# mit-han-lab/distrifuser

Measured on AMD Instinct MI355X. Metric: end-to-end latency (s) per image, SDXL 50-step DDIM, lower is better.
Workload: dtype bf16; 1 GPU; model=sdxl-base (random init), global_batch=1, image=3840x3840, seq_len=230400, scheduler=ddim, steps_per_image=50, parallelism=patch1, mode=corrected_async_gn, cuda_graph=True

## Files before the change

### distrifuser_amd/csrc/attention.hip

```cpp

#include "common.h"
#include "kernels.h"

#include <algorithm>
#include <type_traits>

namespace {

constexpr int QW = 32;
constexpr int KVB = 128;
constexpr bool SPLIT_STAGE = true;

typedef float float4v_ __attribute__((ext_vector_type(4)));
typedef float float16v __attribute__((ext_vector_type(16)));
typedef short short4v __attribute__((ext_vector_type(4)));
typedef __attribute__((address_space(3))) short4v lds_short4v;

template <int DPAD>
__device__ __forceinline__ int v_swz(int t) {
    if constexpr (DPAD % 128 == 0)
        return (t & 3) << 6;
    else if constexpr (DPAD % 64 == 0)
        return ((t >> 1) & 1) << 6;
    else
        return 0;
}

__device__ __forceinline__ uint32_t cvt_pk_bf16(float a, float b) {
    uint32_t r;
    asm("v_cvt_pk_bf16_f32 %0, %1, %2" : "=v"(r) : "v"(a), "v"(b));
    return r;
}

__device__ __forceinline__ void lds_barrier() {
    asm volatile("s_waitcnt lgkmcnt(0)\n\ts_barrier" ::: "memory");
}

__device__ __forceinline__ float half_max(float v) {
    const uint32_t u = __builtin_bit_cast(uint32_t, v);
    const auto r = __builtin_amdgcn_permlane32_swap(u, u, false, false);
    const uint32_t a = r[0], b = r[1];
    float m;
    asm("v_max_f32 %0, %1, %2" : "=v"(m) : "v"(a), "v"(b));
    return m;
}
__device__ __forceinline__ float half_sum(float v) {
    const uint32_t u = __builtin_bit_cast(uint32_t, v);
    const auto r = __builtin_amdgcn_permlane32_swap(u, u, false, false);
    const uint32_t a = r[0], b = r[1];
    return __builtin_bit_cast(float, a) + __builtin_bit_cast(float, b);
}

template <int NW, int DPAD, bool DFULL, bool SPLIT, bool LSE>
__global__ __launch_bounds__(NW * WAVE_SIZE)
__attribute__((amdgpu_waves_per_eu(DPAD == 64 ? 4 : 2))) void flash_attn_kernel(
    std::conditional_t<LSE, FlashAttnLseParams, FlashAttnParams> p, bool off32) {
    constexpr int NT = NW * WAVE_SIZE;
    constexpr int QBLK = QW * NW;
    constexpr int K_ROW = DPAD * 2 + 8;
    constexpr int V_ROW = DPAD * 2;
    constexpr int KS = DPAD / 16;
    constexpr int DT = DPAD / 32;
    constexpr int KCOLS = DPAD / 8;
    constexpr int NLD = KVB * KCOLS / NT;
    static_assert(KVB * KCOLS % NT == 0);
    __shared__ __attribute__((aligned(16))) char k_lds[KVB * K_ROW];
    __shared__ __attribute__((aligned(16))) char v_lds[KVB * V_ROW];

    const int tid = threadIdx.x;
    const int wave = tid / WAVE_SIZE;
    const int lane = tid % WAVE_SIZE;
    const int lo = lane & 31;
    const int hi = lane >> 5;

    const int bh = blockIdx.y;
    const int b = bh / p.H;
    const int h = bh % p.H;
    const int64_t q0 = (int64_t)blockIdx.x * QBLK;

    const int LC = (int)p.LC;
    const int Lkv = (int)(p.NC * p.LC);
    const uint16_t* qbase = p.q + b * p.q_sb + h * p.q_sh;
    const uint16_t* kbase = p.k + b * p.k_sb + h * p.k_sh;
    const uint16_t* vbase = p.v + b * p.v_sb + h * p.v_sh;

    short8 qf[KS];
    const int64_t qrow = q0 + wave * QW + lo;
    const bool qvalid = qrow < p.Lq;
    {
        const uint16_t* qp = qbase + (qvalid ? qrow : (p.Lq - 1)) * p.q_sl;
#pragma unroll
        for (int ks = 0; ks < KS; ++ks) {
            const int d0 = ks * 16 + hi * 8;
            if (DFULL || d0 + 8 <= p.Dh)
                qf[ks] = *reinterpret_cast<const short8*>(qp + d0);
            else
                qf[ks] = short8{0, 0, 0, 0, 0, 0, 0, 0};
        }
    }

    int vrd[DT];
    {
        const int i = lane & 15;
        const int q = i >> 2;
        const int col_b = ((lane >> 4) & 1) * 32 + (i & 3) * 8;
#pragma unroll
        for (int dt = 0; dt < DT; ++dt)
            vrd[dt] = (hi * 8 + q) * V_ROW + ((dt * 64 + col_b) ^ v_swz<DPAD>(q));
    }

    int cur_chunk = 0, cur_tin = 0;
    const char* kcur = reinterpret_cast<const char*>(kbase);
    const char* vcur = reinterpret_cast<const char*>(vbase);
    int tile_lo = 0, tile_hi = 0;
    if constexpr (LSE) {
        const int n_tiles = (Lkv + KVB - 1) / KVB;
        const int n_splits = (int)gridDim.z, split = (int)blockIdx.z;
        tile_lo = (int)((int64_t)split * n_tiles / n_splits);
        tile_hi = (int)((int64_t)(split + 1) * n_tiles / n_splits);
        if (tile_lo > 0) {
            const int tok = tile_lo * KVB;
            cur_chunk = tok / LC;
            cur_tin = tok - cur_chunk * LC;
            kcur = reinterpret_cast<const char*>(kbase + cur_chunk * p.k_sc + cur_tin * p.k_sl);
            vcur = reinterpret_cast<const char*>(vbase + cur_chunk * p.v_sc + cur_tin * p.v_sl);
        }
    }
    uint4 kreg[NLD], vreg[NLD];
    constexpr bool ROWPASS = NT % KCOLS == 0;
    auto stage_row = [&](int i) {
        if constexpr (ROWPASS)
            return tid / KCOLS + i * (NT / KCOLS);
        else
            return (tid + i * NT) / KCOLS;
    };
    auto stage_col = [&](int i) {
        if constexpr (ROWPASS)
            return tid % KCOLS;
        else
            return (tid + i * NT) % KCOLS;
    };
    auto stage_d_ok = [&](int i) { return DFULL || stage_col(i) * 8 + 8 <= p.Dh; };
    const uint32_t koff = (uint32_t)stage_row(0) * ((uint32_t)p.k_sl * 2) + stage_col(0) * 16;
    const uint32_t voff = (uint32_t)stage_row(0) * ((uint32_t)p.v_sl * 2) + stage_col(0) * 16;
    const int k_pass = (NT / KCOLS) * (int)p.k_sl * 2;
    const int v_pass = (NT / KCOLS) * (int)p.v_sl * 2;
    auto tile_rsrc = [](const char* cur) {
        return __builtin_amdgcn_make_buffer_rsrc(const_cast<char*>(cur), 0, 0xFFFFFFFFu,
                                                 0x00020000);
    };
    auto stage_load = [&](int t0, bool full) {
        if (ROWPASS && full && off32 && cur_tin + KVB <= LC) {
            const auto krs = tile_rsrc(kcur);
            const auto vrs = tile_rsrc(vcur);
#pragma unroll
            for (int i = 0; i < NLD; ++i) {
                if constexpr (!DFULL) {
                    kreg[i] = uint4{0, 0, 0, 0};
                    vreg[i] = uint4{0, 0, 0, 0};
                }
                if (stage_d_ok(i)) {
                    kreg[i] = __builtin_bit_cast(
                        uint4, __builtin_amdgcn_raw_buffer_load_b128(
                                   krs, (int)koff, i * k_pass, 0));
                    vreg[i] = __builtin_bit_cast(
                        uint4, __builtin_amdgcn_raw_buffer_load_b128(
                                   vrs, (int)voff, i * v_pass, 0));
                }
            }
        } else {
#pragma unroll
            for (int i = 0; i < NLD; ++i) {
                const int t_local = stage_row(i);
                const int d8 = stage_col(i);
                int tin = cur_tin + t_local;
                int ch = cur_chunk;
                while (tin >= LC) {
                    tin -= LC;
                    ++ch;
                }
                kreg[i] = uint4{0, 0, 0, 0};
                vreg[i] = uint4{0, 0, 0, 0};
                if (stage_d_ok(i) && t0 + t_local < Lkv) {
                    kreg[i] = *reinterpret_cast<const uint4*>(
                        kbase + ch * p.k_sc + tin * p.k_sl + d8 * 8);
                    vreg[i] = *reinterpret_cast<const uint4*>(
                        vbase + ch * p.v_sc + tin * p.v_sl + d8 * 8);
                }
            }
        }
        cur_tin += KVB;
        kcur += KVB * p.k_sl * 2;
        vcur += KVB * p.v_sl * 2;
        if (cur_tin >= LC) {
            do {
                cur_tin -= LC;
                ++cur_chunk;
            } while (cur_tin >= LC);
            kcur = reinterpret_cast<const char*>(kbase + cur_chunk * p.k_sc + cur_tin * p.k_sl);
            vcur = reinterpret_cast<const char*>(vbase + cur_chunk * p.v_sc + cur_tin * p.v_sl);
        }
    };
    auto stage_write = [&]() {
#pragma unroll
        for (int i = 0; i < NLD; ++i) {
            const int t_local = stage_row(i);
            const int d8 = stage_col(i);
            char* kdst = &k_lds[t_local * K_ROW + d8 * 16];
            *reinterpret_cast<uint2*>(kdst) = uint2{kreg[i].x, kreg[i].y};
            *reinterpret_cast<uint2*>(kdst + 8) = uint2{kreg[i].z, kreg[i].w};
            *reinterpret_cast<uint4*>(
                &v_lds[t_local * V_ROW + ((d8 * 16) ^ v_swz<DPAD>(t_local))]) = vreg[i];
        }
    };

    float m_raw = -1e30f;
    float msc = -1e30f;
    float l_run = 0.f;
    float16v ot[DT] = {};
    const float scale2 = p.scale * 1.44269504088896340736f;
    const float defer_raw = 11.0f / scale2;

    auto qk_tile = [&](int st) {
        float16v s = {};
        __builtin_amdgcn_s_setprio(1);
#pragma unroll
        for (int ks = 0; ks < KS; ++ks) {
            const int t = st * 32 + lo;
            const char* ksrc = &k_lds[t * K_ROW + (ks * 16 + hi * 8) * 2];
            const uint2 k0 = *reinterpret_cast<const uint2*>(ksrc);
            const uint2 k1 = *reinterpret_cast<const uint2*>(ksrc + 8);
            const uint4 kk{k0.x, k0.y, k1.x, k1.y};
            const short8 kfrag = __builtin_bit_cast(short8, kk);
            s = __builtin_amdgcn_mfma_f32_32x32x16_bf16(kfrag, qf[ks], s, 0, 0, 0);
        }
        __builtin_amdgcn_s_setprio(0);
        return s;
    };

    auto compute = [&]<int NST, bool MASK>(int t0) {
        float16v s_cur = qk_tile(0);
#pragma unroll
        for (int st = 0; st < NST; ++st) {
            float16v s_nxt;
            if (st + 1 < NST) s_nxt = qk_tile(st + 1);
            const float16v s = s_cur;
            float tm = -1e30f;
            float pv[16];
#pragma unroll
            for (int r = 0; r < 16; ++r) {
                float v = s[r];
                if (MASK) {
                    const int crow = (r & 3) + 8 * (r >> 2) + 4 * hi;
                    if (t0 + st * 32 + crow >= Lkv) v = -1e30f;
                }
                pv[r] = v;
                tm = fmaxf(tm, v);
            }
            tm = half_max(tm);

            if (__any(m_raw == -1e30f || tm > m_raw + defer_raw)) {
                const float m_new = fmaxf(m_raw, tm);
                const float msc_new = m_new * scale2;
                const float corr = __builtin_amdgcn_exp2f(msc - msc_new);
                m_raw = m_new;
                msc = msc_new;
                l_run *= corr;
#pragma unroll
                for (int dt = 0; dt < DT; ++dt)
#pragma unroll
                    for (int r = 0; r < 16; ++r) ot[dt][r] *= corr;
            }
            float tsum = 0.f;
#pragma unroll
            for (int r = 0; r < 16; ++r) {
                pv[r] = __builtin_amdgcn_exp2f(__builtin_fmaf(pv[r], scale2, -msc));
                tsum += pv[r];
            }
            l_run += half_sum(tsum);

            uint32_t w[8];
#pragma unroll
            for (int i = 0; i < 8; ++i) w[i] = cvt_pk_bf16(pv[2 * i], pv[2 * i + 1]);
            short8 pb[2];
#pragma unroll
            for (int kt = 0; kt < 2; ++kt) {
                const auto r0 = __builtin_amdgcn_permlane32_swap(w[4 * kt + 0], w[4 * kt + 2],
                                                                 false, false);
                const auto r1 = __builtin_amdgcn_permlane32_swap(w[4 * kt + 1], w[4 * kt + 3],
                                                                 false, false);
                const uint4 pw{r0[0], r1[0], r0[1], r1[1]};
                pb[kt] = __builtin_bit_cast(short8, pw);
            }

            __builtin_amdgcn_s_setprio(1);
#pragma unroll
            for (int dt = 0; dt < DT; ++dt) {
#pragma unroll
                for (int kt = 0; kt < 2; ++kt) {
                    const char* vsrc = &v_lds[vrd[dt] + (st * 32 + kt * 16) * V_ROW];
                    const short4v v0 =
                        __builtin_amdgcn_ds_read_tr16_b64_v4i16((lds_short4v*)vsrc);
                    const short4v v1 =
                        __builtin_amdgcn_ds_read_tr16_b64_v4i16((lds_short4v*)(vsrc + 4 * V_ROW));
                    const short8 vf = __builtin_shufflevector(v0, v1, 0, 1, 2, 3, 4, 5, 6, 7);
                    ot[dt] = __builtin_amdgcn_mfma_f32_32x32x16_bf16(vf, pb[kt], ot[dt], 0, 0, 0);
                }
            }
            __builtin_amdgcn_s_setprio(0);
            s_cur = s_nxt;
        }
    };

    const int tile0 = LSE ? tile_lo : 0;
    const int n_full = LSE ? min(tile_hi, Lkv / KVB) : Lkv / KVB;
    const int rem = LSE && tile_hi * KVB <= Lkv ? 0 : Lkv % KVB;
    if (Lkv > 0) {
        stage_load(tile0 * KVB, tile0 < n_full);
        stage_write();
        lds_barrier();
    }
    __builtin_amdgcn_s_waitcnt(0x0F70);
    for (int tile = tile0; tile < n_full; ++tile) {
        const int t0 = tile * KVB;
        const bool next_full = tile + 1 < n_full;
        auto load_next = [&]() {
            if (next_full || rem) stage_load(t0 + KVB, next_full);
        };
        if (SPLIT) load_next();
        compute.template operator()<KVB / 32, false>(t0);
        if (next_full || rem) {
            lds_barrier();
            if (!SPLIT) load_next();
            stage_write();
            lds_barrier();
        }
    }
    if (rem == 64)
        compute.template operator()<2, false>(n_full * KVB);
    else if (rem)
        compute.template operator()<KVB / 32, true>(n_full * KVB);

    const float inv = l_run > 0.f ? 1.f / l_run : 0.f;
    if constexpr (LSE) {
        const float lse = l_run > 0.f
                              ? 0.69314718055994530942f * (msc + __builtin_amdgcn_logf(l_run))
                              : -__builtin_inff();
        const int64_t sb = (int64_t)blockIdx.z * p.B + b;
        if (qvalid && hi == 0) p.lse[(sb * p.H + h) * p.Lq + qrow] = lse;
        if (p.o_part != nullptr) {
            float* op32 = p.o_part + (sb * p.Lq + (qvalid ? qrow : 0)) * (p.H * p.Dh) +
                          (int64_t)h * p.Dh;
#pragma unroll
            for (int dt = 0; dt < DT; ++dt) {
#pragma unroll
                for (int g = 0; g < 4; ++g) {
                    const int d0 = dt * 32 + 8 * g + 4 * hi;
                    if (qvalid && (DFULL || d0 + 4 <= p.Dh))
                        *reinterpret_cast<float4*>(op32 + d0) =
                            float4{ot[dt][4 * g] * inv, ot[dt][4 * g + 1] * inv,
                                   ot[dt][4 * g + 2] * inv, ot[dt][4 * g + 3] * inv};
                }
            }
            return;
        }
    }
    uint16_t* op = p.o + ((int64_t)b * p.Lq + (qvalid ? qrow : 0)) * (p.H * p.Dh) +
                   (int64_t)h * p.Dh;
#pragma unroll
    for (int dt = 0; dt < DT; ++dt) {
        uint32_t ow[8];
#pragma unroll
        for (int i = 0; i < 8; ++i) {
            const uint32_t e0 =
                __builtin_bit_cast(uint16_t, __float2bfloat16(ot[dt][2 * i] * inv));
            const uint32_t e1 =
                __builtin_bit_cast(uint16_t, __float2bfloat16(ot[dt][2 * i + 1] * inv));
            ow[i] = e0 | (e1 << 16);
        }
#pragma unroll
        for (int g = 0; g < 4; g += 2) {
            const auto rx = __builtin_amdgcn_permlane32_swap(ow[2 * g], ow[2 * g + 2],
                                                             false, false);
            const auto ry = __builtin_amdgcn_permlane32_swap(ow[2 * g + 1], ow[2 * g + 3],
                                                             false, false);
            const int d0 = dt * 32 + 8 * (g + hi);
            if (qvalid && (DFULL || d0 + 8 <= p.Dh))
                *reinterpret_cast<uint4*>(op + d0) = uint4{rx[0], ry[0], rx[1], ry[1]};
        }
    }
}

}

namespace {

template <bool OUT_BF16>
__global__ __launch_bounds__(256) void merge_attn_kernel(MergeAttnParams p) {
    const int dcols = p.Dh / 8;
    const int64_t idx = (int64_t)blockIdx.x * 256 + threadIdx.x;
    const int64_t rows = (int64_t)p.B * p.Lq * p.H;
    if (idx >= rows * dcols) return;
    const int64_t row = idx / dcols;
    const int dc = (int)(idx - row * dcols);
    const int h = (int)(row % p.H);
    const int64_t bq = row / p.H;
    const int64_t qi = bq % p.Lq;
    const int64_t b = bq / p.Lq;
    const int64_t lse_row = (b * p.H + h) * p.Lq + qi;
    const int64_t lse_ss = (int64_t)p.B * p.H * p.Lq;
    const int64_t o_ss = rows * p.Dh;

    float m = -__builtin_inff();
    for (int s = 0; s < p.S; ++s) m = fmaxf(m, p.lse_parts[s * lse_ss + lse_row]);
    float acc[8] = {};
    float wsum = 0.f;
    if (m > -__builtin_inff()) {
        const float* src = p.o_parts + row * p.Dh + dc * 8;
        for (int s = 0; s < p.S; ++s) {
            const float w = expf(p.lse_parts[s * lse_ss + lse_row] - m);
            const float4 a = *reinterpret_cast<const float4*>(src + s * o_ss);
            const float4 c = *reinterpret_cast<const float4*>(src + s * o_ss + 4);
            if (w > 0.f) {
                wsum += w;
                acc[0] += w * a.x, acc[1] += w * a.y, acc[2] += w * a.z, acc[3] += w * a.w;
                acc[4] += w * c.x, acc[5] += w * c.y, acc[6] += w * c.z, acc[7] += w * c.w;
            }
        }
        const float inv = 1.f / wsum;
#pragma unroll
        for (int j = 0; j < 8; ++j) acc[j] *= inv;
    }
    if (OUT_BF16) {
        uint32_t w[4];
#pragma unroll
        for (int j = 0; j < 4; ++j) {
            const uint32_t e0 = __builtin_bit_cast(uint16_t, __float2bfloat16(acc[2 * j]));
            const uint32_t e1 = __builtin_bit_cast(uint16_t, __float2bfloat16(acc[2 * j + 1]));
            w[j] = e0 | (e1 << 16);
        }
        *reinterpret_cast<uint4*>(static_cast<uint16_t*>(p.out) + row * p.Dh + dc * 8) =
            uint4{w[0], w[1], w[2], w[3]};
    } else {
        float* dst = static_cast<float*>(p.out) + row * p.Dh + dc * 8;
        *reinterpret_cast<float4*>(dst) = float4{acc[0], acc[1], acc[2], acc[3]};
        *reinterpret_cast<float4*>(dst + 4) = float4{acc[4], acc[5], acc[6], acc[7]};
    }
    if (dc == 0 && p.lse != nullptr)
        p.lse[lse_row] = wsum > 0.f ? m + logf(wsum) : -__builtin_inff();
}

}

void launch_merge_attention(const MergeAttnParams& p, hipStream_t stream) {
    const int64_t total = (int64_t)p.B * p.Lq * p.H * (p.Dh / 8);
    if (total == 0) return;
    const dim3 grid((unsigned)((total + 255) / 256));
    if (p.out_bf16)
        merge_attn_kernel<true><<<grid, 256, 0, stream>>>(p);
    else
        merge_attn_kernel<false><<<grid, 256, 0, stream>>>(p);
}

namespace {

template <int DPAD>
bool fits_off32(const FlashAttnParams& p) {
    const int64_t sl = p.k_sl > p.v_sl ? p.k_sl : p.v_sl;
    return sl >= 0 && sl * 2 * KVB + DPAD * 2 <= (int64_t)INT32_MAX;
}

template <int DPAD>
void launch_dpad_lse(const FlashAttnLseParams& p, int splits, hipStream_t stream) {
    constexpr int NW = 8;
    const int qblk = QW * NW;
    dim3 grid((unsigned)((p.Lq + qblk - 1) / qblk), (unsigned)(p.B * p.H), (unsigned)splits);
    dim3 block(NW * WAVE_SIZE);
    const bool off32 = fits_off32<DPAD>(p);
    if (p.Dh == DPAD)
        flash_attn_kernel<NW, DPAD, true, SPLIT_STAGE, true><<<grid, block, 0, stream>>>(p, off32);
    else
        flash_attn_kernel<NW, DPAD, false, SPLIT_STAGE, true><<<grid, block, 0, stream>>>(p, off32);
}

}

template <int DPAD>
static void launch_dpad(const FlashAttnParams& p, hipStream_t stream) {
    constexpr int NW = 8;
    const int qblk = QW * NW;
    dim3 grid((unsigned)((p.Lq + qblk - 1) / qblk), (unsigned)(p.B * p.H));
    dim3 block(NW * WAVE_SIZE);
    const bool off32 = fits_off32<DPAD>(p);
    if (p.Dh == DPAD)
        flash_attn_kernel<NW, DPAD, true, SPLIT_STAGE, false><<<grid, block, 0, stream>>>(p, off32);
    else
        flash_attn_kernel<NW, DPAD, false, SPLIT_STAGE, false><<<grid, block, 0, stream>>>(p, off32);
}

void launch_flash_attention_d64(const FlashAttnParams& p, hipStream_t stream) {
    if (p.Dh <= 64)
        launch_dpad<64>(p, stream);
    else if (p.Dh <= 96)
        launch_dpad<96>(p, stream);
    else if (p.Dh <= 128)
        launch_dpad<128>(p, stream);
    else
        launch_dpad<160>(p, stream);
}

int flash_attention_num_splits(int64_t lkv, int splits) {
    const int64_t tiles = (lkv + KVB - 1) / KVB;
    return (int)std::max<int64_t>(1, std::min<int64_t>(splits, tiles));
}

void launch_flash_attention_lse(const FlashAttnLseParams& p, int splits, hipStream_t stream) {
    splits = flash_attention_num_splits(p.NC * p.LC, splits);
    if (p.Dh <= 64)
        launch_dpad_lse<64>(p, splits, stream);
    else if (p.Dh <= 96)
        launch_dpad_lse<96>(p, splits, stream);
    else if (p.Dh <= 128)
        launch_dpad_lse<128>(p, splits, stream);
    else
        launch_dpad_lse<160>(p, splits, stream);
}

namespace {
__global__ void mfma_probe_kernel(const float* __restrict__ a, const float* __restrict__ b,
                                  float* __restrict__ d) {
    const int lane = threadIdx.x;
    short8 af, bf;
#pragma unroll
    for (int j = 0; j < 8; ++j) {
        af[j] = __builtin_bit_cast(short, __float2bfloat16(a[lane * 8 + j]));
        bf[j] = __builtin_bit_cast(short, __float2bfloat16(b[lane * 8 + j]));
    }
    float4v_ acc = {};
    acc = __builtin_amdgcn_mfma_f32_16x16x32_bf16(af, bf, acc, 0, 0, 0);
#pragma unroll
    for (int r = 0; r < 4; ++r) d[lane * 4 + r] = acc[r];
}

__global__ void mfma_probe32_kernel(const float* __restrict__ a, const float* __restrict__ b,
                                    float* __restrict__ d) {
    const int lane = threadIdx.x;
    short8 af, bf;
#pragma unroll
    for (int j = 0; j < 8; ++j) {
        af[j] = __builtin_bit_cast(short, __float2bfloat16(a[lane * 8 + j]));
        bf[j] = __builtin_bit_cast(short, __float2bfloat16(b[lane * 8 + j]));
    }
    float16v acc = {};
    acc = __builtin_amdgcn_mfma_f32_32x32x16_bf16(af, bf, acc, 0, 0, 0);
#pragma unroll
    for (int r = 0; r < 16; ++r) d[lane * 16 + r] = acc[r];
}
}

void launch_mfma_probe(const float* a, const float* b, float* d, hipStream_t stream) {
    mfma_probe_kernel<<<1, WAVE_SIZE, 0, stream>>>(a, b, d);
}

void launch_mfma_probe32(const float* a, const float* b, float* d, hipStream_t stream) {
    mfma_probe32_kernel<<<1, WAVE_SIZE, 0, stream>>>(a, b, d);
}
```

Measured before the change: 28.36 s/image.

## Widen K LDS row padding for 128-bit reads and defer row-sum reduction

The K tile in LDS now uses a 16-byte row pad so each lane can read its bf16 fragment with one 128-bit load instead of two 64-bit loads, and the stage writes use single 128-bit stores. The rescale test is reduced to one comparison against a precomputed threshold, and the scale constants are forced into scalar registers with readfirstlane. The cross-half row-sum reduction moves out of the inner loop: partial sums accumulate per lane and are combined once at the end. The trade-offs are slightly more LDS use, a changed bank-conflict pattern, and a different floating-point summation order.

```diff
diff --git a/distrifuser_amd/csrc/attention.hip b/distrifuser_amd/csrc/attention.hip
--- a/distrifuser_amd/csrc/attention.hip
+++ b/distrifuser_amd/csrc/attention.hip
@@ -57,7 +57,8 @@
     std::conditional_t<LSE, FlashAttnLseParams, FlashAttnParams> p, bool off32) {
     constexpr int NT = NW * WAVE_SIZE;
     constexpr int QBLK = QW * NW;
-    constexpr int K_ROW = DPAD * 2 + 8;
+    constexpr int K_ROW = DPAD * 2 + 16;
+    static_assert((K_ROW / 16) % 2 == 1);
     constexpr int V_ROW = DPAD * 2;
     constexpr int KS = DPAD / 16;
     constexpr int DT = DPAD / 32;
@@ -108,6 +109,7 @@
         for (int dt = 0; dt < DT; ++dt)
             vrd[dt] = (hi * 8 + q) * V_ROW + ((dt * 64 + col_b) ^ v_swz<DPAD>(q));
     }
+    const int krd = lo * K_ROW + hi * 16;
 
     int cur_chunk = 0, cur_tin = 0;
     const char* kcur = reinterpret_cast<const char*>(kbase);
@@ -206,9 +208,7 @@
         for (int i = 0; i < NLD; ++i) {
             const int t_local = stage_row(i);
             const int d8 = stage_col(i);
-            char* kdst = &k_lds[t_local * K_ROW + d8 * 16];
-            *reinterpret_cast<uint2*>(kdst) = uint2{kreg[i].x, kreg[i].y};
-            *reinterpret_cast<uint2*>(kdst + 8) = uint2{kreg[i].z, kreg[i].w};
+            *reinterpret_cast<uint4*>(&k_lds[t_local * K_ROW + d8 * 16]) = kreg[i];
             *reinterpret_cast<uint4*>(
                 &v_lds[t_local * V_ROW + ((d8 * 16) ^ v_swz<DPAD>(t_local))]) = vreg[i];
         }
@@ -216,22 +216,23 @@
 
     float m_raw = -1e30f;
     float msc = -1e30f;
+    float thr = -1e30f;
     float l_run = 0.f;
     float16v ot[DT] = {};
-    const float scale2 = p.scale * 1.44269504088896340736f;
-    const float defer_raw = 11.0f / scale2;
+    auto uniform = [](float x) {
+        return __builtin_bit_cast(
+            float, __builtin_amdgcn_readfirstlane(__builtin_bit_cast(int, x)));
+    };
+    const float scale2 = uniform(p.scale * 1.44269504088896340736f);
+    const float defer_raw = uniform(11.0f / scale2);
 
     auto qk_tile = [&](int st) {
         float16v s = {};
         __builtin_amdgcn_s_setprio(1);
 #pragma unroll
         for (int ks = 0; ks < KS; ++ks) {
-            const int t = st * 32 + lo;
-            const char* ksrc = &k_lds[t * K_ROW + (ks * 16 + hi * 8) * 2];
-            const uint2 k0 = *reinterpret_cast<const uint2*>(ksrc);
-            const uint2 k1 = *reinterpret_cast<const uint2*>(ksrc + 8);
-            const uint4 kk{k0.x, k0.y, k1.x, k1.y};
-            const short8 kfrag = __builtin_bit_cast(short8, kk);
+            const short8 kfrag =
+                *reinterpret_cast<const short8*>(&k_lds[krd + st * 32 * K_ROW + ks * 32]);
             s = __builtin_amdgcn_mfma_f32_32x32x16_bf16(kfrag, qf[ks], s, 0, 0, 0);
         }
         __builtin_amdgcn_s_setprio(0);
@@ -259,25 +260,25 @@
             }
             tm = half_max(tm);
 
-            if (__any(m_raw == -1e30f || tm > m_raw + defer_raw)) {
+            if (__any(tm > thr)) {
                 const float m_new = fmaxf(m_raw, tm);
                 const float msc_new = m_new * scale2;
                 const float corr = __builtin_amdgcn_exp2f(msc - msc_new);
                 m_raw = m_new;
                 msc = msc_new;
+                thr = m_new + defer_raw;
                 l_run *= corr;
 #pragma unroll
                 for (int dt = 0; dt < DT; ++dt)
 #pragma unroll
                     for (int r = 0; r < 16; ++r) ot[dt][r] *= corr;
             }
-            float tsum = 0.f;
 #pragma unroll
             for (int r = 0; r < 16; ++r) {
                 pv[r] = __builtin_amdgcn_exp2f(__builtin_fmaf(pv[r], scale2, -msc));
-                tsum += pv[r];
-            }
-            l_run += half_sum(tsum);
+                l_run += pv[r];
+            }
+            asm volatile("" : "+v"(l_run));
 
             uint32_t w[8];
 #pragma unroll
@@ -341,6 +342,7 @@
     else if (rem)
         compute.template operator()<KVB / 32, true>(n_full * KVB);
 
+    l_run = half_sum(l_run);
     const float inv = l_run > 0.f ? 1.f / l_run : 0.f;
     if constexpr (LSE) {
         const float lse = l_run > 0.f
```

After: 27.90 s/image (median of 3 runs). Within noise of the previous version (-1.6%).
